# cunningham-lab/cyclic-gps

Measured on AMD Instinct MI355X. Metric: block-tridiag solve+log-det (mahal_and_det) algorithmic GB/s vs HBM roofline, N=2^20 d=4 on one GPU, N=2^24 d=4 time-axis sharded on several; solves/s alongside, higher is better.
Workload: dtype f64; 1 GPU; BASELINE config 2: mahal_and_det on ONE SPD block-tridiagonal system, N=1048576 block rows (1048576 per GPU), d=4, conditioned bidiagonal-factor generator seed 1234; rows_total=1048576, rows_per_gpu=1048576, d=4, algorithmic_bytes=301989776, parallelism=single GPU, algo=tile-fused

## Files before the change

### cyclic-gps_amd/csrc/cgps_tile.h

```cpp
#pragma once
#include <cstdlib>
#include <map>
#include <mutex>
#include <utility>
#include <type_traits>

#include "cgps_level.h"
#include "cgps_plan.h"
#include "cgps_leg.h"

namespace cgps {
#include "cgps_tile_leg.h"

template <typename T, int D>
struct LdsTile {
  static constexpr int DD = D * D;
  static constexpr int VN = Vec16<T>::N;
  static constexpr int G = (DD % VN == 0) ? DD / VN : 0;
  static constexpr bool SWZ = G >= 2 && (G & (G - 1)) == 0;
  T* R;
  T* Oc;
  T* y;
  static __device__ __forceinline__ int key(int row) { return (row ^ (row >> 3) ^ (row >> 6) ^ (row >> 9)) & (G - 1); }

// ... 280 lines not shown
          }
        }
      }
      CGPS_STAMP(1);
      __syncthreads();
      CGPS_STAMP(2);
      if (act) {
        if (role == 0) {
          LT::store_blk(t.R, e, W);
          store_vec<T, D>(t.y + e * D, wv);
        } else if (role == 1) {
          LT::store_blk(t.R, o, W);
          store_vec<T, D>(t.y + o * D, wv);
        } else if (role == 2) {
          LT::template store_rows<0, DH>(t.Oc, e - s + 1, W);
        } else {
          LT::template store_rows<DH, D>(t.Oc, e - s + 1, W);
        }
      }
      __syncthreads();
      CGPS_STAMP(3);
      ++stamp_pass;
    }
  }
  return levels;
}

template <typename T>
__device__ __forceinline__ void store_wt(T* p, T v) {
  __hip_atomic_store(p, v, __ATOMIC_RELAXED, __HIP_MEMORY_SCOPE_AGENT);
}
template <bool COH, typename T>
__device__ __forceinline__ T load_coh(const T* p) {
  if constexpr (COH) return __hip_atomic_load(const_cast<T*>(p), __ATOMIC_RELAXED, __HIP_MEMORY_SCOPE_AGENT);
  else return *p;
}
template <bool COH, typename T>
__device__ __forceinline__ typename Vec16<T>::type load16_coh(const T* p) {
  using V = typename Vec16<T>::type;
  if constexpr (COH) {
    unsigned long long* q = reinterpret_cast<unsigned long long*>(const_cast<T*>(p));
    unsigned long long w[2];
    w[0] = __hip_atomic_load(q, __ATOMIC_RELAXED, __HIP_MEMORY_SCOPE_AGENT);
    w[1] = __hip_atomic_load(q + 1, __ATOMIC_RELAXED, __HIP_MEMORY_SCOPE_AGENT);
    V v;
    __builtin_memcpy(&v, w, 16);
    return v;
  } else {
    return *reinterpret_cast<const V*>(p);
  }
}

constexpr int FOLD_SLOTS = 1024;
#ifndef CGPS_FOLD_GROUP
#define CGPS_FOLD_GROUP 16
#endif
constexpr int FOLD_GROUP = CGPS_FOLD_GROUP;
constexpr int FOLD_MAX_GROUPS = 64;
static __device__ unsigned int g_fold_counter[FOLD_SLOTS][1 + FOLD_MAX_GROUPS];

template <typename T, int D> constexpr int record_rcmax() { return (D == 8 || (sizeof(T) == 8 && D == 6)) ? 1 : 4; }

template <typename T, int D>
struct RecordLayout {
  static constexpr int DD = D * D;
  static constexpr int STRIDE = record_stride(D);
  static constexpr int RS = 0, CS = DD, DRA = 2 * DD, YS = 3 * DD, DYA = 3 * DD + D;
};


template <typename T, int D>
__device__ __forceinline__ void collect_left_updates(LdsTile<T, D>& t, int levels, T (&dRa)[D][D], T (&dya)[D]) {
  for (int l = 0; l < levels; ++l) {
    const int slot = (1 << l) - 1;
    T P[D][D], p[D];
    LdsTile<T, D>::load_blk(t.R, slot, P);
    load_vec<T, D>(t.y + slot * D, p);
#pragma unroll
    for (int i = 0; i < D; ++i) {
      dya[i] -= p[i];
#pragma unroll
      for (int j = 0; j <= i; ++j) dRa[i][j] -= P[i][j];
    }
  }
}

constexpr int FAIL_LATE = 0x40000000;
__device__ __forceinline__ int fail_code(bool early, bool any, int64_t row) {
  const int r = (int)(row < (int64_t)(FAIL_LATE - 2) ? row : (int64_t)(FAIL_LATE - 2)) + 1;
  return early ? r : (any ? (r | FAIL_LATE) : 0);
}
template <int NT>
__device__ __forceinline__ void write_partial(double mah, double logp, int failrow_plus1, double* __restrict__ partial,
                                              double* red, int* sfail) {
  if (failrow_plus1) atomicMin(sfail, failrow_plus1);
  block_sum2<NT>(mah, logp, red);
  if constexpr (NT <= 64) __syncthreads();
  if (threadIdx.x == 0) {
    double* p = partial;
    const int f = *sfail;
    store_wt(p + 0, mah);
    store_wt(p + 1, logp);
    store_wt(p + 2, (f == 0x7fffffff) ? 0.0 : (double)f);
    store_wt(p + 3, 0.0);
  }
}
// ... 105 lines not shown
    for (int l = 0; l < levels; ++l) {
      const int slot = (1 << l) - 1;
      dra -= elem(t.R, slot);
      dyv -= t.y[slot * D + i];
    }
    T* r = rec_out;
    store_wt(r + RL::RS + tid, elem(t.R, n_real - 1));
    store_wt(r + RL::CS + tid, elem(t.Oc, 0));
    store_wt(r + RL::DRA + tid, dra);
    if (j == 0) {
      store_wt(r + RL::YS + i, t.y[(n_real - 1) * D + i]);
      store_wt(r + RL::DYA + i, dyv);
    }
  }
}

template <typename T, int D, int NTILE, int NT>
struct StageSmem {
  static constexpr int DD = D * D;
  LdsTile<T, D> t;
  double* red;
  T* xch;
  int* sfail;
  __device__ __forceinline__ StageSmem(char* smem) {
    t.carve(smem, NTILE);
    char* tail = smem + ((((size_t)NTILE * (2 * DD + D) + DD) * sizeof(T) + 15) & ~(size_t)15);
    red = reinterpret_cast<double*>(tail);
    xch = reinterpret_cast<T*>(red + 2 * (NT / 64));
    sfail = reinterpret_cast<int*>(xch + (NT / 64) * (DD + D));
  }
};


template <typename T, int D> constexpr int stage1_row_group() {
  if (sizeof(T) == 8 && (D == 3 || D == 5)) return 2;
  return 1;
}
template <typename T, int D> constexpr int stage1_min_waves() {
  return ((sizeof(T) == 8 && D <= 4) || (sizeof(T) == 4 && D <= 5)) ? 2 : 1;
}
struct FoldArgs {
  int slot;
  void* group_records;
  double* out2;
  int* info;
  void* shard_record;
  double* shard_partial;
  int rows_per_lane;
  int pair_slot;
  size_t pair_ws_stride;
  const unsigned char* obs_pattern;
  int obs_entries;
};
template <typename T, int D, int NTILE, int NT, bool FINAL, bool INL = false>
__device__ __forceinline__ void record_reduce_body(char* smem, unsigned tile_index, const T* __restrict__ rin, int64_t n,
                                                   int rc, T* __restrict__ rout, double* __restrict__ partial_out,
                                                   const double* __restrict__ partial_in, int64_t n_partial,
                                                   double* __restrict__ out2, int* __restrict__ info,
                                                   int64_t rows_per_record, int64_t N, int64_t rstride, int64_t pstride);
template <typename T, int D, int NW, bool ONE_PER_CU>
__device__ __forceinline__ void fold_record_stages(char* smem, int* last_flag, T* __restrict__ rec, double* __restrict__ partial,
                                                   const FoldArgs& fold, int64_t rows_per_tile, int64_t N) {
  const int tid = threadIdx.x;
    constexpr bool COH = ONE_PER_CU && (D * D) % Vec16<T>::N == 0;
    using RL = RecordLayout<T, D>;
    const unsigned grp = blockIdx.x / FOLD_GROUP, ngrp = (gridDim.x + FOLD_GROUP - 1) / FOLD_GROUP;
    const unsigned gsize = (grp + 1 < ngrp) ? (unsigned)FOLD_GROUP : gridDim.x - grp * FOLD_GROUP;
    auto arrive = [&](unsigned int* ctr, unsigned expected) {
      if (tid < 64) {
        asm volatile("s_waitcnt vmcnt(0)" ::: "memory");
        if (tid == 0) {
          const bool last = atomicInc(ctr, expected - 1u) == expected - 1u;
          *last_flag = last ? 1 : 0;
          if (!COH && last) {
            __builtin_amdgcn_fence(__ATOMIC_ACQUIRE, "agent");
            asm volatile("s_waitcnt vmcnt(0)" ::: "memory");
          }
        }
      }
      __syncthreads();
      return *last_flag != 0;
    };
    T* grec = reinterpret_cast<T*>(fold.group_records);
    double* gpartial = partial + PARTIAL_STRIDE * (size_t)gridDim.x;
    const bool lead = arrive(&g_fold_counter[fold.slot][1 + grp], gsize);
    CGPS_KSTAMP(4);
    if (gridDim.x == 1) {
      record_reduce_body<T, D, FOLD_MAX_GROUPS, NW, true, COH>(smem, 0u, rec, (int64_t)1, 1, (T*)nullptr, (double*)nullptr,
                                                               partial, (int64_t)1, fold.out2, fold.info, rows_per_tile, N,
                                                               (int64_t)RL::STRIDE, (int64_t)PARTIAL_STRIDE);
      return;
    }
    if (lead) {
      record_reduce_body<T, D, FOLD_GROUP, NW, false, COH>(smem, grp, rec, (int64_t)gridDim.x, 1, grec, gpartial,
                                                           (const double*)nullptr, (int64_t)0, (double*)nullptr,
                                                           (int*)nullptr, rows_per_tile, N, (int64_t)RL::STRIDE,
                                                           (int64_t)PARTIAL_STRIDE);
      CGPS_KSTAMP(5);
      const bool fin = arrive(&g_fold_counter[fold.slot][0], ngrp);
      CGPS_KSTAMP(6);
      if (fin) {
        if (fold.shard_record != nullptr)
          record_reduce_body<T, D, FOLD_MAX_GROUPS, NW, false, COH>(smem, 0u, grec, (int64_t)ngrp, 1,
                                                                    reinterpret_cast<T*>(fold.shard_record), fold.shard_partial,
                                                                    partial, (int64_t)gridDim.x + ngrp, (double*)nullptr,
                                                                    (int*)nullptr, rows_per_tile * FOLD_GROUP, N,
                                                                    (int64_t)RL::STRIDE, (int64_t)PARTIAL_STRIDE);
        else
          record_reduce_body<T, D, FOLD_MAX_GROUPS, NW, true, COH>(smem, 0u, grec, (int64_t)ngrp, 1, (T*)nullptr,
                                                                   (double*)nullptr, partial, (int64_t)gridDim.x + ngrp,
                                                                   fold.out2, fold.info, rows_per_tile * FOLD_GROUP, N,
                                                                   (int64_t)RL::STRIDE, (int64_t)PARTIAL_STRIDE);
        CGPS_KSTAMP(7);
      }
    }
}

template <typename T, int D, int CT, int NT, int NW = NT, bool FOLD = false, int SRC = 0>
__global__ __launch_bounds__(NW, (NW > NT ? 1 : stage1_min_waves<T, D>())) void chunk_reduce_kernel(const T* __restrict__ Rg, const T* __restrict__ Og,
                                                          const T* __restrict__ yg, int64_t N,
                                                          const T* __restrict__ Oleft,
                                                          T* __restrict__ rec, double* __restrict__ partial,
                                                          FoldArgs fold) {
  constexpr int DD = D * D;
  extern __shared__ __attribute__((aligned(16))) char smem[];
  StageSmem<T, D, NT, NW> sm(smem);
  const int tid = threadIdx.x;
  CGPS_KSTAMP(0);
  if (tid == 0) *sm.sfail = 0x7fffffff;
  const int C = CT > 0 ? CT : fold.rows_per_lane;
  if constexpr (SRC >= 1) {
    if (blockIdx.y == 1) {
      Oleft = nullptr;
      yg = nullptr;
      rec = reinterpret_cast<T*>(reinterpret_cast<char*>(rec) + fold.pair_ws_stride);
      partial = reinterpret_cast<double*>(reinterpret_cast<char*>(partial) + fold.pair_ws_stride);
      fold.group_records = reinterpret_cast<char*>(fold.group_records) + fold.pair_ws_stride;
      fold.slot = fold.pair_slot;
      fold.out2 += 2;
      fold.info += 1;
    }
  }
  const int64_t lane0 = (int64_t)blockIdx.x * NT;
  const int64_t gl = lane0 + tid;
  int64_t r0 = gl * C, rE = gl * C + C;
  if (tid >= NT) r0 = N;
  const bool whole_chunk = rE <= N;
  const bool whole_chunk_and_next = rE <= N - 1;
  if (rE > N) rE = N;
  const int L = r0 < N ? (int)(rE - r0) : 0;
  PivotLog pl;
  double mah = 0.0;
// ... 403 lines not shown
    (void)hipFuncSetAttribute(reinterpret_cast<const void*>(&chunk_reduce_ml_kernel<T, D, Cfg::C, Cfg::NT1, Cfg::LPR, true>),
                              hipFuncAttributeMaxDynamicSharedMemorySize, lds1);
  }
  else if constexpr (Cfg::ALWAYS_WIDE) {
    const int ldsw = (int)stage_lds_bytes<T, D>(Cfg::NG1, 2 * Cfg::NT1);
    (void)hipFuncSetAttribute(reinterpret_cast<const void*>(&chunk_reduce_kernel<T, D, Cfg::C, Cfg::NT1, 2 * Cfg::NT1>),
                              hipFuncAttributeMaxDynamicSharedMemorySize, ldsw);
    (void)hipFuncSetAttribute(reinterpret_cast<const void*>(&chunk_reduce_kernel<T, D, Cfg::C, Cfg::NT1, 2 * Cfg::NT1, true>),
                              hipFuncAttributeMaxDynamicSharedMemorySize, ldsw);
    (void)hipFuncSetAttribute(reinterpret_cast<const void*>(&chunk_reduce_kernel<T, D, 0, Cfg::NT1, 2 * Cfg::NT1, true>),
                              hipFuncAttributeMaxDynamicSharedMemorySize, ldsw);
    (void)hipFuncSetAttribute(reinterpret_cast<const void*>(&chunk_reduce_kernel<T, D, 0, Cfg::NT1, 2 * Cfg::NT1, true, 1>),
                              hipFuncAttributeMaxDynamicSharedMemorySize, ldsw);
  } else {
    (void)hipFuncSetAttribute(reinterpret_cast<const void*>(&chunk_reduce_kernel<T, D, 0, Cfg::NT1, Cfg::NT1, true>),
                              hipFuncAttributeMaxDynamicSharedMemorySize, lds1);
    (void)hipFuncSetAttribute(reinterpret_cast<const void*>(&chunk_reduce_kernel<T, D, 0, Cfg::NT1, Cfg::NT1, true, 1>),
                              hipFuncAttributeMaxDynamicSharedMemorySize, lds1);
    (void)hipFuncSetAttribute(reinterpret_cast<const void*>(&chunk_reduce_kernel<T, D, Cfg::C, Cfg::NT1>),
                              hipFuncAttributeMaxDynamicSharedMemorySize, lds1);
    (void)hipFuncSetAttribute(reinterpret_cast<const void*>(&chunk_reduce_kernel<T, D, Cfg::C, Cfg::NT1, Cfg::NT1, true>),
                              hipFuncAttributeMaxDynamicSharedMemorySize, lds1);
    if constexpr (stage1_min_waves<T, D>() == 2) {
      (void)hipFuncSetAttribute(reinterpret_cast<const void*>(&chunk_reduce_kernel<T, D, Cfg::C, Cfg::NT1, 2 * Cfg::NT1>),
                                hipFuncAttributeMaxDynamicSharedMemorySize,
                                (int)stage_lds_bytes<T, D>(Cfg::NG1, 2 * Cfg::NT1));
      (void)hipFuncSetAttribute(reinterpret_cast<const void*>(&chunk_reduce_kernel<T, D, Cfg::C, Cfg::NT1, 2 * Cfg::NT1, true>),
                                hipFuncAttributeMaxDynamicSharedMemorySize,
                                (int)stage_lds_bytes<T, D>(Cfg::NG1, 2 * Cfg::NT1));
      (void)hipFuncSetAttribute(reinterpret_cast<const void*>(&chunk_reduce_kernel<T, D, 0, Cfg::NT1, 2 * Cfg::NT1, true>),
                                hipFuncAttributeMaxDynamicSharedMemorySize,
                                (int)stage_lds_bytes<T, D>(Cfg::NG1, 2 * Cfg::NT1));
    }
    (void)hipFuncSetAttribute(reinterpret_cast<const void*>(&chunk_reduce_kernel<T, D, 8, Cfg::NT1>),
                              hipFuncAttributeMaxDynamicSharedMemorySize, lds1);
    (void)hipFuncSetAttribute(reinterpret_cast<const void*>(&chunk_reduce_kernel<T, D, 8, Cfg::NT1, Cfg::NT1, true>),
                              hipFuncAttributeMaxDynamicSharedMemorySize, lds1);
    (void)hipFuncSetAttribute(reinterpret_cast<const void*>(&chunk_reduce_kernel<T, D, 4, Cfg::NT1>),
                              hipFuncAttributeMaxDynamicSharedMemorySize, lds1);
    (void)hipFuncSetAttribute(reinterpret_cast<const void*>(&chunk_reduce_kernel<T, D, 4, Cfg::NT1, Cfg::NT1, true>),
                              hipFuncAttributeMaxDynamicSharedMemorySize, lds1);
    (void)hipFuncSetAttribute(reinterpret_cast<const void*>(&chunk_reduce_kernel<T, D, 1, Cfg::NT1>),
                              hipFuncAttributeMaxDynamicSharedMemorySize, lds1);
    (void)hipFuncSetAttribute(reinterpret_cast<const void*>(&chunk_reduce_kernel<T, D, 1, Cfg::NT1, Cfg::NT1, true>),
                              hipFuncAttributeMaxDynamicSharedMemorySize, lds1);
  }
  (void)hipFuncSetAttribute(reinterpret_cast<const void*>(&record_reduce_kernel<T, D, Cfg::NTILE3, Cfg::NT3, false>),
                            hipFuncAttributeMaxDynamicSharedMemorySize, lds3);
  (void)hipFuncSetAttribute(reinterpret_cast<const void*>(&record_reduce_kernel<T, D, Cfg::NTILE3, Cfg::NT3, true>),
                            hipFuncAttributeMaxDynamicSharedMemorySize, lds3);
  });
}

static int fold_slot_for(const void* ws) {
  static std::mutex mu;
  static std::map<std::pair<int, const void*>, int> slots;
  static std::pair<int, const void*> owner[FOLD_SLOTS];
  static unsigned long long last_use[FOLD_SLOTS];
  static unsigned long long tick = 0;
  int dev = 0;
  (void)hipGetDevice(&dev);
  const std::pair<int, const void*> key{dev, ws};
  std::lock_guard<std::mutex> lock(mu);
  auto it = slots.find(key);
  int s;
  if (it != slots.end()) {
    s = it->second;
  } else if ((int)slots.size() < FOLD_SLOTS) {
    s = (int)slots.size();
    slots.emplace(key, s);
    owner[s] = key;
  } else {
    s = 0;
    for (int k = 1; k < FOLD_SLOTS; ++k)
      if (last_use[k] < last_use[s]) s = k;
    slots.erase(owner[s]);
    slots.emplace(key, s);
    owner[s] = key;
  }
  last_use[s] = ++tick;
  return s;
}
static hipError_t fold_reset_counters(hipStream_t st) {
  void* p = nullptr;
  hipError_t e = hipGetSymbolAddress(&p, HIP_SYMBOL(g_fold_counter));
  if (e != hipSuccess) return e;
  return hipMemsetAsync(p, 0, sizeof(unsigned int) * FOLD_SLOTS * (1 + FOLD_MAX_GROUPS), st);
}
inline bool fold_final_enabled() {
  static const bool on = [] { const char* e = getenv("CGPS_NO_FOLD"); return !(e && e[0] == '1'); }();
  return on;
}

inline int long_chunk_target_tiles() {
  static const int v = [] {
    const char* e = getenv("CGPS_S1_LONG");
    if (e && e[0] == '0') return 0;
    const char* t = getenv("CGPS_S1_TILES");
    const int n = t ? atoi(t) : 0;
    return n > 0 ? n : (int)STAGE1_SMALL_TILES;
  }();
  return v;
}
inline bool long_chunk_narrow() {
  static const bool on = [] { const char* e = getenv("CGPS_S1_NARROW"); return e && e[0] == '1'; }();
  return on;
}
inline int long_chunk_rows_per_lane(int64_t N, int lanes, int c_full, int block_bytes) {
  const int tiles = long_chunk_target_tiles();
  if (tiles <= 0) return 0;
  static const int forced = [] { const char* e = getenv("CGPS_S1_C"); return e ? atoi(e) : 0; }();
  if (forced > 0 && forced % 4 == 0 && (N + (int64_t)forced * lanes - 1) / ((int64_t)forced * lanes) <= 1024 &&
      N > (int64_t)forced * lanes)
    return forced;
  const int64_t per_round = (int64_t)tiles * lanes;
  int64_t c = (N + per_round - 1) / per_round;
  c = (c + 3) & ~(int64_t)3;
  if (c <= c_full || c > (1 << 20)) return 0;
  if (c * block_bytes > 2048 && c * block_bytes < 16384) return 0;
  return (int)c;
}

template <typename T, int D>
int run_tile_mahal_logdet(const T* Rs, const T* Os, const T* x, int64_t N, char* ws, size_t ws_bytes, double* out2,
                          int* info, hipStream_t st, hipEvent_t ev_start = nullptr, hipEvent_t ev_stop = nullptr,
                          const T* Oleft = nullptr, T* shard_record = nullptr, double* shard_partial = nullptr) {
  using Cfg = TileCfg<T, D>;
  using RL = RecordLayout<T, D>;
  static_assert(Cfg::ROWS1 == tile_rows1(D, sizeof(T)), "the workspace is sized for other stage-1 tiles than the kernels take");
  const cgps_host::TileWs w = cgps_host::tile_ws(N, D, sizeof(T));
  if (ws_bytes < w.total) return -1;
  const int clong = (Cfg::LPR > 1 || !fold_final_enabled()) ? 0 : long_chunk_rows_per_lane(N, Cfg::NG1, Cfg::C, (int)(D * D * sizeof(T)));
  const int csel = clong > 0 ? clong : ((Cfg::LPR > 1 || Cfg::ALWAYS_WIDE) ? Cfg::C : stage1_rows_per_lane(N, Cfg::C, Cfg::NT1));
  const int64_t rows_per_tile = (int64_t)csel * Cfg::NG1;
// ... 197 lines not shown
```

### cyclic-gps_amd/csrc/dev_bench.hip

```cpp
#include <hip/hip_runtime.h>

#include <cmath>
#include <cstdio>
#include <cstdlib>
#include <vector>

#define CGPS_FIN_STAMPS 1
#ifndef DEVB_D
#define DEVB_D 4
#endif
#ifndef DEVB_T
#define DEVB_T double
#endif
#include "cgps_tile.h"

using namespace cgps;

template <typename T, int D>
__device__ __forceinline__ void set_identity(T (&A)[D][D]) {
#pragma unroll
  for (int i = 0; i < D; ++i)
#pragma unroll
    for (int j = 0; j < D; ++j) A[i][j] = (i == j) ? T(1) : T(0);
}
// ... 145 lines not shown
        for (int b = 0; b <= a; ++b) { T v = (a == b) ? (T)2.5 + (T)0.2 * rnd() : (T)0.1 * rnd(); R[a][b] = v; R[b][a] = v; }
        for (int b = 0; b < D; ++b) O[a][b] = (T)0.3 * rnd();
        y[a] = rnd();
      }
      LdsTile<T, D>::store_blk(sm.t.R, tid, R);
      LdsTile<T, D>::store_blk(sm.t.Oc, tid, O);
      store_vec<T, D>(sm.t.y + tid * D, y);
    }
    __syncthreads();
    const long long t0 = wall_clock64();
    tile_cr<T, D, NTHR, MW>(sm.t, n_real, pl, mah, fail);
    const long long t1 = wall_clock64();
    __syncthreads();
    acc += t1 - t0;
  }
  double logp = pl.value();
  block_sum2<NTHR>(mah, logp, sm.red);
  if (tid == 0) {
    ticks[blockIdx.x] = acc;
    sums[2 * blockIdx.x] = mah;
    sums[2 * blockIdx.x + 1] = logp;
  }
}

template <int NTHR, int MW>
void run_tilecr(int grid, hipStream_t st) {
  const size_t lds = stage_lds_bytes<DEVB_T, DEVB_D>(256, NTHR);
  CK(hipFuncSetAttribute(reinterpret_cast<const void*>(&tilecr_bench_kernel<NTHR, MW>),
                         hipFuncAttributeMaxDynamicSharedMemorySize, (int)lds));
  long long* ticks;
  double* sums;
  CK(hipMalloc(&ticks, grid * sizeof(long long)));
  CK(hipMalloc(&sums, 2 * grid * sizeof(double)));
  const int reps = 50;
  printf("tile_cr NTHR=%d MW=%d grid=%d :", NTHR, MW, grid);
  double prev = 0;
  for (int n_real : {2, 4, 8, 16, 32, 64, 128, 256}) {
    hipLaunchKernelGGL((tilecr_bench_kernel<NTHR, MW>), dim3(grid), dim3(NTHR), lds, st, n_real, reps, ticks, sums);
    CK(hipStreamSynchronize(st));
    std::vector<long long> h(grid);
    std::vector<double> hs(2 * grid);
    CK(hipMemcpy(h.data(), ticks, grid * sizeof(long long), hipMemcpyDeviceToHost));
    CK(hipMemcpy(hs.data(), sums, 2 * grid * sizeof(double), hipMemcpyDeviceToHost));
    double avg = 0;
    for (auto v : h) avg += (double)v;
    avg = avg / grid / reps * 10.0;
    printf("  n=%d: %.0f ns (+%.0f)", n_real, avg, avg - prev);
    if (n_real == 256) printf("  [check %.10g %.10g]", hs[0], hs[1]);
    prev = avg;
  }
  printf("\n");
  CK(hipFree(ticks));
  CK(hipFree(sums));
}

template <typename F>
float time_ms(F&& launch, int reps, hipStream_t st) {
  hipEvent_t a, b;
  CK(hipEventCreate(&a));
  CK(hipEventCreate(&b));
  launch();
  CK(hipStreamSynchronize(st));
  CK(hipEventRecord(a, st));
  for (int i = 0; i < reps; ++i) launch();
  CK(hipEventRecord(b, st));
  CK(hipEventSynchronize(b));
  float ms = 0;
  CK(hipEventElapsedTime(&ms, a, b));
  CK(hipGetLastError());
  return ms / reps;
}

template <typename T, int D, int C, int NT>
void run_chunk_variants(const T* R, const T* O, const T* y, int64_t N, double* out, hipStream_t st, double bytes) {
  const int64_t tiles = (N + (int64_t)C * NT - 1) / ((int64_t)C * NT);
  float a = time_ms([&] { hipLaunchKernelGGL((loads_only_kernel<T, D, C, NT>), dim3((unsigned)tiles), dim3(NT), 0, st, R, O, y, N, out); }, 20, st);
  float b = time_ms([&] { hipLaunchKernelGGL((chunk_only_kernel<T, D, C, NT>), dim3((unsigned)tiles), dim3(NT), 0, st, R, O, y, N, out); }, 20, st);
  printf("C=%2d NT=%3d tiles=%6lld : loads-only %7.2f us (%5.2f TB/s)   chunk-only %7.2f us (%5.2f TB/s)\n", C, NT,
         (long long)tiles, a * 1e3, bytes / (a * 1e-3) / 1e12, b * 1e3, bytes / (b * 1e-3) / 1e12);
}

int main(int argc, char** argv) {
  using T = double;
  constexpr int D = DEVB_D;
  const int lg = argc > 1 ? atoi(argv[1]) : 20;
  const int64_t N = (int64_t)1 << lg;
  if (argc > 2 && atoi(argv[2]) == 2) {
    hipStream_t s2;
    CK(hipStreamCreate(&s2));
    T *R2, *O2, *y2;
    CK(hipMalloc(&R2, N * D * D * sizeof(T)));
    CK(hipMalloc(&O2, N * D * D * sizeof(T)));
    CK(hipMalloc(&y2, N * D * sizeof(T)));
    hipLaunchKernelGGL((gen_kernel<T, D>), dim3((unsigned)((N + 255) / 256)), dim3(256), 0, s2, R2, O2, y2, N);
    const size_t wsb = cgps_host::tile_ws(N, D, sizeof(T)).total;
    char* ws;
    double* out2;
    int* info;
    CK(hipMalloc(&ws, wsb));
    CK(hipMalloc(&out2, 16));
    CK(hipMalloc(&info, 4));
    for (int mode = (argc > 3 ? atoi(argv[3]) : 0); mode < 2; ++mode) {
      setenv("CGPS_NO_FOLD", mode == 0 ? "1" : "0", 1);
      for (int it = 0; it < 30; ++it) {
        hipEvent_t ea, eb;
        CK(hipEventCreate(&ea));
        CK(hipEventCreate(&eb));
        CK(hipEventRecord(ea, s2));
        int rc = run_tile_mahal_logdet<T, D>(R2, O2, y2, N, ws, wsb, out2, info, s2);
        CK(hipEventRecord(eb, s2));
        CK(hipStreamSynchronize(s2));
        float ms;
        CK(hipEventElapsedTime(&ms, ea, eb));
        long long st[16];
        CK(hipMemcpyFromSymbol(st, HIP_SYMBOL(g_fin_stamps), sizeof(st)));
        double o[2];
        CK(hipMemcpy(o, out2, 16, hipMemcpyDeviceToHost));
        if (it >= 28) {
          static long long ks[512][12];
          CK(hipMemcpyFromSymbol(ks, HIP_SYMBOL(g_k_stamps), sizeof(ks)));
          long long t0 = ks[0][0];
          for (int b = 0; b < 256; ++b) t0 = ks[b][0] < t0 ? ks[b][0] : t0;
          static int xcc[512];
          CK(hipMemcpyFromSymbol(xcc, HIP_SYMBOL(g_k_xcc), sizeof(xcc)));
          double sx[8] = {0}, mx[8] = {0};
          int cx[8] = {0};
          for (int b = 0; b < 256; ++b) {
            const int x = xcc[b] & 7;
            const double d = (ks[b][1] - t0) * 0.01;
            sx[x] += d; cx[x]++; mx[x] = d > mx[x] ? d : mx[x];
          }
          printf("   stream end per XCD (avg/max us):");
          for (int x = 0; x < 8; ++x) printf(" [%d: n=%d %.1f/%.1f]", x, cx[x], cx[x] ? sx[x] / cx[x] : 0.0, mx[x]);
          printf("\n   stream end by block index (us):");
          for (int b = 0; b < 256; b += 17) printf(" b%d:%.1f", b, (ks[b][1] - t0) * 0.01);
          printf("\n");
          const char* names[10] = {"start", "streamed", "tile reduced+emitted", "partial written", "arrived(group)",
                                   "group reduced", "arrived(top)", "final done", "rows staged in LDS", "tile_cr done"};
          for (int k = 0; k < 10; ++k) {
            long long lo = 1LL << 62, hi = 0;
            int cnt = 0;
            for (int b = 0; b < 256; ++b) {
              if (ks[b][k] < t0) continue;
              lo = ks[b][k] < lo ? ks[b][k] : lo;
              hi = ks[b][k] > hi ? ks[b][k] : hi;
              ++cnt;
            }
            if (cnt) printf("   %-22s first %.2f us  last %.2f us  (%d workgroups)\n", names[k], (lo - t0) * 0.01, (hi - t0) * 0.01, cnt);
          }
        }
        if (it >= 27)
          printf("mode %s rc %d: op %.1f us | final: loads %.2f  lds-stores %.2f  reduce %.2f  last-row %.2f  sums+write %.2f  total %.2f us  [%.10g %.10g]\n",
                 mode == 0 ? "two launches" : "folded", rc, ms * 1e3, (st[1] - st[0]) * 0.01, (st[2] - st[1]) * 0.01,
                 (st[3] - st[2]) * 0.01, (st[4] - st[3]) * 0.01, (st[5] - st[4]) * 0.01, (st[5] - st[0]) * 0.01, o[0], o[1]);
      }
      break;
    }
    return 0;
  }
  if (argc > 2 && atoi(argv[2]) == 1) {
    hipStream_t s2;
    CK(hipStreamCreate(&s2));
    for (int grid : {1, 256}) {
      run_tilecr<256, 1>(grid, s2);
      run_tilecr<256, 2>(grid, s2);
      run_tilecr<256, 4>(grid, s2);
      run_tilecr<512, 1>(grid, s2);
      run_tilecr<512, 2>(grid, s2);
      run_tilecr<512, 4>(grid, s2);
    }
    return 0;
  }
  hipStream_t st;
  CK(hipStreamCreate(&st));
  T *R, *O, *y;
  double* out;
  CK(hipMalloc(&R, N * D * D * sizeof(T)));
  CK(hipMalloc(&O, N * D * D * sizeof(T)));
  CK(hipMalloc(&y, N * D * sizeof(T)));
  CK(hipMalloc(&out, 4096));
  hipLaunchKernelGGL((gen_kernel<T, D>), dim3((unsigned)((N + 255) / 256)), dim3(256), 0, st, R, O, y, N);
  CK(hipStreamSynchronize(st));
  const double bytes = ((2.0 * N - 1) * D * D + N * D) * sizeof(T);
  printf("N=2^%d d=%d fp64  algorithmic bytes %.1f MB\n", lg, D, bytes / 1e6);
  run_mfma_probe();

  {
    const int64_t n16 = N * D * D * sizeof(T) / 16;
    float ms = time_ms([&] {
      hipLaunchKernelGGL(coalesced_read_kernel, dim3(2048), dim3(256), 0, st, (const double2*)R, n16, out);
      hipLaunchKernelGGL(coalesced_read_kernel, dim3(2048), dim3(256), 0, st, (const double2*)O, n16, out);
    }, 20, st);
    printf("coalesced read of R+O (2 launches): %7.2f us  (%5.2f TB/s)\n", ms * 1e3, 2.0 * n16 * 16 / (ms * 1e-3) / 1e12);
  }
  run_chunk_variants<T, D, 4, 256>(R, O, y, N, out, st, bytes);
  run_chunk_variants<T, D, 8, 256>(R, O, y, N, out, st, bytes);
  run_chunk_variants<T, D, 16, 256>(R, O, y, N, out, st, bytes);
  run_chunk_variants<T, D, 8, 128>(R, O, y, N, out, st, bytes);
  run_chunk_variants<T, D, 8, 64>(R, O, y, N, out, st, bytes);
  run_chunk_variants<T, D, 16, 64>(R, O, y, N, out, st, bytes);
  run_chunk_variants<T, D, 32, 64>(R, O, y, N, out, st, bytes);

  return 0;
}
```

Before: 4375 GB/s.

## Fold f64 d=4 record reduction stages in one wave using registers and DPP

For double precision with d=4 and at most 256 workgroups, the cross-workgroup fold of per-tile records now runs in a single 64-lane wave. The block-tridiagonal cyclic reduction over up to 16 records is done in registers with MFMA 4x4 ops and DPP row rotations, replacing the LDS-staged multi-wave reduction. The aim is to shorten the serial tail latency of the last-arriving workgroups, at the cost of considerable new index-mapping complexity. An environment variable falls back to the LDS path, and a microbenchmark mode is added.

```diff
diff --git a/cyclic-gps_amd/csrc/cgps_tile.h b/cyclic-gps_amd/csrc/cgps_tile.h
--- a/cyclic-gps_amd/csrc/cgps_tile.h
+++ b/cyclic-gps_amd/csrc/cgps_tile.h
@@ -356,6 +356,7 @@
 }
 
 constexpr int FOLD_SLOTS = 1024;
+constexpr int FOLD_SLOT_LDS_STAGES = 1 << 16;
 #ifndef CGPS_FOLD_GROUP
 #define CGPS_FOLD_GROUP 16
 #endif
@@ -567,6 +568,7 @@
   const unsigned char* obs_pattern;
   int obs_entries;
 };
+#include "cgps_tile_rec.h"
 template <typename T, int D, int NTILE, int NT, bool FINAL, bool INL = false>
 __device__ __forceinline__ void record_reduce_body(char* smem, unsigned tile_index, const T* __restrict__ rin, int64_t n,
                                                    int rc, T* __restrict__ rout, double* __restrict__ partial_out,
@@ -581,6 +583,51 @@
     using RL = RecordLayout<T, D>;
     const unsigned grp = blockIdx.x / FOLD_GROUP, ngrp = (gridDim.x + FOLD_GROUP - 1) / FOLD_GROUP;
     const unsigned gsize = (grp + 1 < ngrp) ? (unsigned)FOLD_GROUP : gridDim.x - grp * FOLD_GROUP;
+    const int slot = fold.slot & (FOLD_SLOT_LDS_STAGES - 1);
+    if constexpr (std::is_same<T, double>::value && D == 4 && FOLD_GROUP == fold_reg::MAX_RECORDS) {
+      if (gridDim.x <= FOLD_GROUP * fold_reg::MAX_RECORDS && !(fold.slot & FOLD_SLOT_LDS_STAGES)) {
+        if (tid >= 64) return;
+        int lane = tid;
+        asm volatile("" : "+v"(lane));
+        auto arrive1 = [&](unsigned int* ctr, unsigned expected) {
+          asm volatile("s_waitcnt vmcnt(0)" ::: "memory");
+          int last = 0;
+          if (lane == 0) last = atomicInc(ctr, expected - 1u) == expected - 1u;
+          last = __builtin_amdgcn_readfirstlane(last);
+          if (!COH && last) {
+            __builtin_amdgcn_fence(__ATOMIC_ACQUIRE, "agent");
+            asm volatile("s_waitcnt vmcnt(0)" ::: "memory");
+          }
+          return last != 0;
+        };
+        const double* recd = reinterpret_cast<const double*>(rec);
+        double* grecd = reinterpret_cast<double*>(fold.group_records);
+        double* gpart = partial + PARTIAL_STRIDE * (size_t)gridDim.x;
+        const bool lead1 = arrive1(&g_fold_counter[slot][1 + grp], gsize);
+        CGPS_KSTAMP(4);
+        if (!lead1) return;
+        const bool single = gridDim.x == 1;
+#pragma unroll 1
+        for (int top = single ? 1 : 0; top < 2; ++top) {
+          const bool t1 = top != 0;
+          const double* rin = t1 ? (single ? recd : grecd) : recd + (size_t)grp * FOLD_GROUP * RL::STRIDE;
+          double* rout = t1 ? reinterpret_cast<double*>(fold.shard_record) : grecd + (size_t)grp * RL::STRIDE;
+          double* pout = t1 ? fold.shard_partial : gpart + PARTIAL_STRIDE * (size_t)grp;
+          const int n = t1 ? (single ? 1 : (int)ngrp) : (int)gsize;
+          const int np = t1 ? (single ? 1 : (int)(gridDim.x + ngrp)) : 0;
+          record_stage_reg<COH>(lane, t1 && fold.shard_record == nullptr, rin, n, rout, pout, t1 ? partial : nullptr, np,
+                                fold.out2, fold.info, t1 ? (int64_t)0 : (int64_t)grp * FOLD_GROUP,
+                                (t1 && !single) ? rows_per_tile * FOLD_GROUP : rows_per_tile, N);
+          if (t1) break;
+          CGPS_KSTAMP(5);
+          const bool fin1 = arrive1(&g_fold_counter[slot][0], ngrp);
+          CGPS_KSTAMP(6);
+          if (!fin1) return;
+        }
+        CGPS_KSTAMP(7);
+        return;
+      }
+    }
     auto arrive = [&](unsigned int* ctr, unsigned expected) {
       if (tid < 64) {
         asm volatile("s_waitcnt vmcnt(0)" ::: "memory");
@@ -598,7 +645,7 @@
     };
     T* grec = reinterpret_cast<T*>(fold.group_records);
     double* gpartial = partial + PARTIAL_STRIDE * (size_t)gridDim.x;
-    const bool lead = arrive(&g_fold_counter[fold.slot][1 + grp], gsize);
+    const bool lead = arrive(&g_fold_counter[slot][1 + grp], gsize);
     CGPS_KSTAMP(4);
     if (gridDim.x == 1) {
       record_reduce_body<T, D, FOLD_MAX_GROUPS, NW, true, COH>(smem, 0u, rec, (int64_t)1, 1, (T*)nullptr, (double*)nullptr,
@@ -612,7 +659,7 @@
                                                            (int*)nullptr, rows_per_tile, N, (int64_t)RL::STRIDE,
                                                            (int64_t)PARTIAL_STRIDE);
       CGPS_KSTAMP(5);
-      const bool fin = arrive(&g_fold_counter[fold.slot][0], ngrp);
+      const bool fin = arrive(&g_fold_counter[slot][0], ngrp);
       CGPS_KSTAMP(6);
       if (fin) {
         if (fold.shard_record != nullptr)
@@ -1122,6 +1169,11 @@
   });
 }
 
+inline bool fold_reg_enabled() {
+  static const bool on = [] { const char* e = getenv("CGPS_FOLD_REG"); return !(e && e[0] == '0'); }();
+  return on;
+}
+
 static int fold_slot_for(const void* ws) {
   static std::mutex mu;
   static std::map<std::pair<int, const void*>, int> slots;
@@ -1149,7 +1201,7 @@
     owner[s] = key;
   }
   last_use[s] = ++tick;
-  return s;
+  return fold_reg_enabled() ? s : (s | FOLD_SLOT_LDS_STAGES);
 }
 static hipError_t fold_reset_counters(hipStream_t st) {
   void* p = nullptr;
diff --git a/cyclic-gps_amd/csrc/cgps_tile_rec.h b/cyclic-gps_amd/csrc/cgps_tile_rec.h
--- /dev/null
+++ b/cyclic-gps_amd/csrc/cgps_tile_rec.h
@@ -0,0 +1,332 @@
+#pragma once
+
+namespace fold_reg {
+constexpr int MAX_RECORDS = 16;
+constexpr int set_of_residue(int m) { return m == 1 ? 2 : (m == 2 ? 1 : m); }
+constexpr int reg_set(int p) { return set_of_residue(p & 3); }
+constexpr int reg_blk(int p) { return p >> 2; }
+constexpr int position(int u, int b) { return 4 * b + set_of_residue(u); }
+constexpr int owner_lane(int p, int r, int c) { return 16 * r + 4 * reg_blk(p) + c; }
+constexpr int levels(int n) { int l = 0; while ((1 << l) < n) ++l; return l; }
+constexpr bool eliminated(int p, int l, int n) { return p < n - 1 && ((p + 1) & ((2 << l) - 1)) == (1 << l); }
+constexpr bool survivor(int p, int l) { return ((p + 1) & ((2 << l) - 1)) == 0; }
+constexpr bool right_is_tail(int p, int l, int n) { return p + (1 << l) >= n - 1; }
+constexpr bool left_is_outside(int p, int l) { return p < (1 << l); }
+constexpr int left_source(int p, int l) { return p - (1 << l); }
+constexpr int right_source(int p, int l) { return p + (1 << l); }
+constexpr int chains(int l) { return l == 0 ? 2 : 1; }
+constexpr int chain_set(int l, int j) { return l == 0 ? j : (l == 1 ? 2 : 3); }
+constexpr int right_set(int l, int u) { return l == 0 ? u + 2 : 3; }
+constexpr int right_rot(int l, int u) { return l == 2 ? 4 : (l == 3 ? 8 : 0); }
+constexpr int left_set(int l, int u) { return l == 0 ? 3 - u : 3; }
+constexpr int left_rot(int l, int u) { return (l == 0 && u == 1) ? 0 : (l == 3 ? 8 : 12); }
+constexpr int last_eliminated(int l, int n) { return ((n - 1 - (1 << l)) / (2 << l)) * (2 << l) + (1 << l) - 1; }
+}
+
+#ifdef __HIPCC__
+template <int ROT>
+__device__ __forceinline__ double row_rot_f64(double v) {
+  static_assert(ROT >= 1 && ROT <= 15, "row_ror:1..15");
+  const int lo = __builtin_amdgcn_mov_dpp(__double2loint(v), 0x120 + ROT, 0xf, 0xf, false);
+  const int hi = __builtin_amdgcn_mov_dpp(__double2hiint(v), 0x120 + ROT, 0xf, 0xf, false);
+  return __hiloint2double(hi, lo);
+}
+__device__ __forceinline__ double sum_over_b(double v) {
+  v += row_rot_f64<4>(v);
+  return v + row_rot_f64<8>(v);
+}
+
+template <int U>
+struct RecElim {
+  double GGt[U], Gx[U], FFt[U], Fx[U], FGt[U], GFt[U], X[U], piv[U];
+  bool f[U];
+};
+template <int U, bool PRODUCTS = true>
+__device__ __forceinline__ void rec_eliminate(int r, double ident, double (&A)[U], const double (&Ol)[U],
+                                              const double (&OrT)[U], const double (&Y)[U], RecElim<U>& o) {
+  double B[U];
+#pragma unroll
+  for (int u = 0; u < U; ++u) { B[u] = ident; o.piv[u] = 1.0; o.f[u] = false; }
+#pragma unroll
+  for (int kk = 0; kk < 4; ++kk) {
+    const double sel = (r == kk) ? 1.0 : 0.0;
+    double rowA[U], rowB[U], p[U], col[U];
+#pragma unroll
+    for (int u = 0; u < U; ++u) {
+      rowA[u] = mfma444(sel, A[u], 0.0);
+      rowB[u] = mfma444(sel, B[u], 0.0);
+    }
+#pragma unroll
+    for (int u = 0; u < U; ++u) {
+      if (kk == 0) { p[u] = quad_bcast_f64<0>(rowA[u]); col[u] = quad_bcast_f64<0>(A[u]); }
+      else if (kk == 1) { p[u] = quad_bcast_f64<1>(rowA[u]); col[u] = quad_bcast_f64<1>(A[u]); }
+      else if (kk == 2) { p[u] = quad_bcast_f64<2>(rowA[u]); col[u] = quad_bcast_f64<2>(A[u]); }
+      else { p[u] = quad_bcast_f64<3>(rowA[u]); col[u] = quad_bcast_f64<3>(A[u]); }
+      o.f[u] = o.f[u] || !(p[u] > 0.0);
+      o.piv[u] *= p[u];
+    }
+    double rs[U];
+#pragma unroll
+    for (int u = 0; u < U; ++u) rs[u] = rsqrt_fast(p[u]);
+#pragma unroll
+    for (int u = 0; u < U; ++u) {
+      const double lik = col[u] * rs[u];
+      const double ra = rowA[u] * rs[u], rb = rowB[u] * rs[u];
+      if (r > kk) {
+        A[u] = __builtin_fma(-lik, ra, A[u]);
+        B[u] = __builtin_fma(-lik, rb, B[u]);
+      } else if (r == kk) {
+        B[u] = rb;
+      }
+    }
+  }
+  double Um[U], Gt[U], Ft[U];
+#pragma unroll
+  for (int u = 0; u < U; ++u) Um[u] = mfma444(B[u], ident, 0.0);
+#pragma unroll
+  for (int u = 0; u < U; ++u) {
+    o.X[u] = mfma444(Um[u], Y[u], 0.0);
+    if constexpr (PRODUCTS) {
+      Gt[u] = mfma444(Um[u], Ol[u], 0.0);
+      Ft[u] = mfma444(Um[u], OrT[u], 0.0);
+    }
+  }
+  if constexpr (PRODUCTS) {
+#pragma unroll
+    for (int u = 0; u < U; ++u) {
+      o.GGt[u] = mfma444(Gt[u], Gt[u], 0.0);
+      o.Gx[u] = mfma444(Gt[u], o.X[u], 0.0);
+      o.FFt[u] = mfma444(Ft[u], Ft[u], 0.0);
+      o.Fx[u] = mfma444(Ft[u], o.X[u], 0.0);
+      o.FGt[u] = mfma444(Ft[u], Gt[u], 0.0);
+      o.GFt[u] = mfma444(Gt[u], Ft[u], 0.0);
+    }
+  }
+}
+
+struct RecStage {
+  double R[4], Y[4], CL[4], CRt[4];
+  double RK, YK, CLK;
+  double dra, dya;
+  double mah;
+  PivotLog pl;
+  int fcode;
+};
+
+template <int L>
+__device__ __forceinline__ void rec_stage_level(RecStage& t, int K, int b, int r, int c, double ident, int64_t rec0,
+                                                int64_t rows_per_record, int64_t N) {
+  namespace fr = fold_reg;
+  constexpr int S = 1 << L, NU = fr::chains(L), MASK = 2 * S - 1;
+  double A[NU], Ol[NU], OrT[NU], Yv[NU];
+  bool act[NU], spec[NU];
+#pragma unroll
+  for (int j = 0; j < NU; ++j) {
+    const int u = fr::chain_set(L, j), p = fr::position(u, b);
+    act[j] = ((p + 1) & MASK) == S && p < K;
+    spec[j] = act[j] && p + S >= K;
+    A[j] = act[j] ? t.R[u] : ident;
+    Ol[j] = act[j] ? t.CL[u] : 0.0;
+    OrT[j] = act[j] ? t.CRt[u] : 0.0;
+    Yv[j] = act[j] ? t.Y[u] : 0.0;
+  }
+  RecElim<NU> e;
+  rec_eliminate<NU>(r, ident, A, Ol, OrT, Yv, e);
+#pragma unroll
+  for (int j = 0; j < NU; ++j) {
+    t.mah += e.X[j] * e.X[j];
+    if (act[j] && r == 0 && c == 0) t.pl.mul(e.piv[j]);
+    if (act[j] && e.f[j]) {
+      int64_t frow = (rec0 + fr::position(fr::chain_set(L, j), b) + 1) * rows_per_record;
+      frow = (frow < N ? frow : N) - 1;
+      const int code = fail_code(false, true, frow);
+      t.fcode = code < t.fcode ? code : t.fcode;
+    }
+  }
+  if (fr::last_eliminated(L, K + 1) + S >= K) {
+    double tR = 0.0, tY = 0.0, tC = 0.0;
+#pragma unroll
+    for (int j = 0; j < NU; ++j) {
+      tR += spec[j] ? e.FFt[j] : 0.0;
+      tY += spec[j] ? e.Fx[j] : 0.0;
+      tC += spec[j] ? e.FGt[j] : 0.0;
+    }
+    t.RK -= sum_over_b(tR);
+    t.YK -= sum_over_b(tY);
+    t.CLK = -sum_over_b(tC);
+  }
+  if (b == fr::reg_blk(S - 1)) {
+    t.dra += e.GGt[0];
+    t.dya += e.Gx[0];
+  }
+  if constexpr (L == 0) {
+    static_assert(fr::right_set(0, 0) == 2 && fr::right_set(0, 1) == 3 && fr::left_set(0, 1) == 2 && fr::left_set(0, 0) == 3, "");
+    static_assert(fr::right_rot(0, 0) == 0 && fr::right_rot(0, 1) == 0 && fr::left_rot(0, 1) == 0, "");
+    constexpr int ROT = fr::left_rot(0, 0);
+    const double gR = row_rot_f64<ROT>(e.GGt[0]), gY = row_rot_f64<ROT>(e.Gx[0]), gC = row_rot_f64<ROT>(e.GFt[0]);
+    t.R[2] -= e.FFt[0];
+    t.Y[2] -= e.Fx[0];
+    t.CL[2] = -e.FGt[0];
+    t.R[2] -= e.GGt[1];
+    t.Y[2] -= e.Gx[1];
+    if (fr::position(2, b) + S < K) t.CRt[2] = -e.GFt[1];
+    t.R[3] -= e.FFt[1];
+    t.Y[3] -= e.Fx[1];
+    t.CL[3] = -e.FGt[1];
+    if (b < 3) {
+      t.R[3] -= gR;
+      t.Y[3] -= gY;
+      if (fr::position(3, b) + S < K) t.CRt[3] = -gC;
+    }
+  } else if constexpr (L == 1) {
+    static_assert(fr::right_set(1, 2) == 3 && fr::left_set(1, 2) == 3 && fr::right_rot(1, 2) == 0, "");
+    constexpr int ROT = fr::left_rot(1, 2);
+    const double gR = row_rot_f64<ROT>(e.GGt[0]), gY = row_rot_f64<ROT>(e.Gx[0]), gC = row_rot_f64<ROT>(e.GFt[0]);
+    t.R[3] -= e.FFt[0];
+    t.Y[3] -= e.Fx[0];
+    t.CL[3] = -e.FGt[0];
+    if (b < 3) {
+      t.R[3] -= gR;
+      t.Y[3] -= gY;
+      if (fr::position(3, b) + S < K) t.CRt[3] = -gC;
+    }
+  } else if constexpr (L == 2) {
+    static_assert(fr::right_set(2, 3) == 3 && fr::left_set(2, 3) == 3, "");
+    constexpr int ROTL = fr::right_rot(2, 3), ROTR = fr::left_rot(2, 3);
+    const double fR = row_rot_f64<ROTL>(e.FFt[0]), fY = row_rot_f64<ROTL>(e.Fx[0]), fC = row_rot_f64<ROTL>(e.FGt[0]);
+    const double gR = row_rot_f64<ROTR>(e.GGt[0]), gY = row_rot_f64<ROTR>(e.Gx[0]), gC = row_rot_f64<ROTR>(e.GFt[0]);
+    if (b == 1) {
+      t.R[3] -= fR;
+      t.Y[3] -= fY;
+      t.CL[3] = -fC;
+      t.R[3] -= gR;
+      t.Y[3] -= gY;
+      if (fr::position(3, b) + S < K) t.CRt[3] = -gC;
+    }
+  }
+}
+
+__device__ __forceinline__ void rec_wave_reduce(double& a, double& b2, int& m) {
+#pragma unroll
+  for (int off = 32; off > 0; off >>= 1) {
+    a += __shfl_down(a, off, 64);
+    b2 += __shfl_down(b2, off, 64);
+    const int o = __shfl_down(m, off, 64);
+    m = o < m ? o : m;
+  }
+}
+
+constexpr int REC_STAGE_MAX_PARTIALS = 320;
+template <bool COH>
+__device__ __forceinline__ void record_stage_reg(int lane, bool FINAL, const double* rin, int n, double* rout,
+                                                 double* partial_out, const double* partial_in,
+                                                 int n_partial, double* out2, int* info,
+                                                 int64_t rec0, int64_t rows_per_record, int64_t N) {
+  using RL = RecordLayout<double, 4>;
+  namespace fr = fold_reg;
+  const int b = (lane >> 2) & 3, r = lane >> 4, c = lane & 3;
+  const int el = 4 * r + c, elT = 4 * c + r;
+  const double ident = (r == c) ? 1.0 : 0.0;
+  const bool c0 = (c == 0);
+  const int K = n - 1;
+  CGPS_FSTAMP(0);
+  double lR[4], lU[4], lC[4], lCr[4], lY[4], lYu[4];
+#pragma unroll
+  for (int u = 0; u < 4; ++u) {
+    const int p = fr::position(u, b);
+    const bool ok = p < K;
+    const double* q = rin + (size_t)(ok ? p : 0) * RL::STRIDE;
+    const double* q1 = rin + (size_t)(ok ? p + 1 : 0) * RL::STRIDE;
+    lR[u] = load_coh<COH>(q + RL::RS + el);
+    lU[u] = load_coh<COH>(q1 + RL::DRA + el);
+    lC[u] = load_coh<COH>(q + RL::CS + el);
+    lCr[u] = load_coh<COH>(q1 + RL::CS + elT);
+    lY[u] = load_coh<COH>(q + RL::YS + r);
+    lYu[u] = load_coh<COH>(q1 + RL::DYA + r);
+  }
+  const double* qk = rin + (size_t)K * RL::STRIDE;
+  const double kR = load_coh<COH>(qk + RL::RS + el), kC = load_coh<COH>(qk + RL::CS + el), kY = load_coh<COH>(qk + RL::YS + r);
+  const double oR = load_coh<COH>(rin + RL::DRA + el), oY = load_coh<COH>(rin + RL::DYA + r);
+  constexpr int PIT = REC_STAGE_MAX_PARTIALS / 64;
+  double pm[PIT], pg[PIT], pf[PIT];
+#pragma unroll
+  for (int it = 0; it < PIT; ++it) {
+    const int i = lane + 64 * it;
+    const bool ok = partial_in != nullptr && i < n_partial;
+    const double* p = (partial_in != nullptr ? partial_in : partial_out) + (size_t)PARTIAL_STRIDE * (ok ? i : 0);
+    pm[it] = ok ? load_coh<COH>(p) : 0.0;
+    pg[it] = ok ? load_coh<COH>(p + 1) : 0.0;
+    pf[it] = ok ? load_coh<COH>(p + 2) : 0.0;
+  }
+  CGPS_FSTAMP(1);
+  RecStage t;
+#pragma unroll
+  for (int u = 0; u < 4; ++u) {
+    const bool ok = fr::position(u, b) < K;
+    t.R[u] = ok ? lR[u] + lU[u] : ident;
+    t.Y[u] = (ok && c0) ? lY[u] + lYu[u] : 0.0;
+    t.CL[u] = ok ? lC[u] : 0.0;
+    t.CRt[u] = ok ? lCr[u] : 0.0;
+  }
+  t.RK = kR;
+  t.YK = c0 ? kY : 0.0;
+  t.CLK = kC;
+  t.dra = 0.0;
+  t.dya = 0.0;
+  t.mah = 0.0;
+  t.fcode = 0x7fffffff;
+  CGPS_FSTAMP(2);
+  if (K >= 1) rec_stage_level<0>(t, K, b, r, c, ident, rec0, rows_per_record, N);
+  if (K >= 2) rec_stage_level<1>(t, K, b, r, c, ident, rec0, rows_per_record, N);
+  if (K >= 4) rec_stage_level<2>(t, K, b, r, c, ident, rec0, rows_per_record, N);
+  if (K >= 8) rec_stage_level<3>(t, K, b, r, c, ident, rec0, rows_per_record, N);
+  CGPS_FSTAMP(3);
+  if (FINAL) {
+    double A[1] = {t.RK}, Z[1] = {0.0}, Yv[1] = {t.YK};
+    RecElim<1> e;
+    rec_eliminate<1, false>(r, ident, A, Z, Z, Yv, e);
+    if (b == 0) t.mah += e.X[0] * e.X[0];
+    if (lane == 0) t.pl.mul(e.piv[0]);
+    if (e.f[0]) {
+      const int code = fail_code(false, true, N - 1);
+      t.fcode = code < t.fcode ? code : t.fcode;
+    }
+    CGPS_FSTAMP(4);
+  } else {
+    const double dra = oR - sum_over_b(t.dra), dya = oY - sum_over_b(t.dya);
+    if (b == 0) {
+      store_wt(rout + RL::RS + el, t.RK);
+      store_wt(rout + RL::CS + el, t.CLK);
+      store_wt(rout + RL::DRA + el, dra);
+      if (c0) {
+        store_wt(rout + RL::YS + r, t.YK);
+        store_wt(rout + RL::DYA + r, dya);
+      }
+    }
+  }
+  double mah = t.mah, logp = t.pl.value();
+  int fcode = t.fcode;
+#pragma unroll
+  for (int it = 0; it < PIT; ++it) {
+    mah += pm[it];
+    logp += pg[it];
+    if (pf[it] != 0.0 && (int)pf[it] < fcode) fcode = (int)pf[it];
+  }
+  rec_wave_reduce(mah, logp, fcode);
+  if (lane == 0) {
+    const bool ok = (fcode == 0x7fffffff);
+    if (FINAL) {
+      const double poison = __builtin_nan("");
+      out2[0] = ok ? mah : poison;
+      out2[1] = ok ? logp : poison;
+      *info = ok ? 0 : (fcode & ~FAIL_LATE);
+    } else {
+      store_wt(partial_out + 0, mah);
+      store_wt(partial_out + 1, logp);
+      store_wt(partial_out + 2, ok ? 0.0 : (double)fcode);
+      store_wt(partial_out + 3, 0.0);
+    }
+  }
+  CGPS_FSTAMP(5);
+}
+#endif
diff --git a/cyclic-gps_amd/csrc/dev_bench.hip b/cyclic-gps_amd/csrc/dev_bench.hip
--- a/cyclic-gps_amd/csrc/dev_bench.hip
+++ b/cyclic-gps_amd/csrc/dev_bench.hip
@@ -221,6 +221,107 @@
   printf("\n");
   CK(hipFree(ticks));
   CK(hipFree(sums));
+}
+
+template <bool REG, bool FINAL>
+__global__ __launch_bounds__(512) void record_stage_bench_kernel(const double* rec, int n, int reps, double* rout, double* pout,
+                                                                 const double* pin, int n_partial, double* out2, int* info,
+                                                                 long long* ticks) {
+  extern __shared__ __attribute__((aligned(16))) char smem[];
+  using RL = RecordLayout<double, 4>;
+  long long acc = 0;
+  for (int rep = 0; rep < reps; ++rep) {
+    __syncthreads();
+    const long long t0 = wall_clock64();
+    if constexpr (REG) {
+      if (threadIdx.x < 64)
+        record_stage_reg<true>((int)threadIdx.x, FINAL, rec, n, rout, pout, FINAL ? pin : nullptr, FINAL ? n_partial : 0, out2, info,
+                                      0, 4096, (int64_t)n * 4096);
+    } else {
+      record_reduce_body<double, 4, (FINAL ? FOLD_MAX_GROUPS : FOLD_GROUP), 512, FINAL, true>(smem, 0u, rec, (int64_t)n, 1, rout, pout, FINAL ? pin : nullptr,
+                                                                  FINAL ? (int64_t)n_partial : 0, out2, info, 4096,
+                                                                  (int64_t)n * 4096, (int64_t)RL::STRIDE, (int64_t)PARTIAL_STRIDE);
+    }
+    asm volatile("s_waitcnt vmcnt(0)" ::: "memory");
+    const long long t1 = wall_clock64();
+    acc += t1 - t0;
+  }
+  if (threadIdx.x == 0) ticks[0] = acc;
+}
+
+template <bool REG, bool FINAL>
+static void run_record_stage(const double* rec, int n, double* rout, double* pout, const double* pin, int n_partial, double* out2,
+                             int* info, long long* ticks, hipStream_t st) {
+  using RL = RecordLayout<double, 4>;
+  const size_t lds = stage_lds_bytes<double, 4>(FOLD_MAX_GROUPS, 512);
+  const int reps = 200;
+  for (int pass = 0; pass < 2; ++pass)
+    hipLaunchKernelGGL((record_stage_bench_kernel<REG, FINAL>), dim3(1), dim3(512), lds, st, rec, n, reps, rout, pout, pin, n_partial,
+                       out2, info, ticks);
+  CK(hipStreamSynchronize(st));
+  long long t;
+  CK(hipMemcpy(&t, ticks, sizeof(t), hipMemcpyDeviceToHost));
+  double r[RL::STRIDE], p[4], o[2];
+  int inf;
+  CK(hipMemcpy(r, rout, sizeof(r), hipMemcpyDeviceToHost));
+  CK(hipMemcpy(p, pout, sizeof(p), hipMemcpyDeviceToHost));
+  CK(hipMemcpy(o, out2, sizeof(o), hipMemcpyDeviceToHost));
+  CK(hipMemcpy(&inf, info, sizeof(inf), hipMemcpyDeviceToHost));
+  double cs = 0;
+  for (int i = 0; i < RL::STRIDE; ++i) cs += r[i] * (1 + i);
+  if (FINAL)
+    printf("  %-9s top stage   n=%2d (+%3d partial results): %6.0f ns   [out2 %.15g %.15g info %d]\n", REG ? "registers" : "LDS", n,
+           n_partial, (double)t / reps * 10.0, o[0], o[1], inf);
+  else
+    printf("  %-9s group stage n=%2d: %6.0f ns   [record checksum %.15g partial %.15g %.15g %g]\n", REG ? "registers" : "LDS", n,
+           (double)t / reps * 10.0, cs, p[0], p[1], p[2]);
+}
+
+static void run_record_stages(hipStream_t st) {
+  using RL = RecordLayout<double, 4>;
+  constexpr int NREC = 16, NPART = 272;
+  std::vector<double> h((size_t)NREC * RL::STRIDE), hp((size_t)NPART * PARTIAL_STRIDE, 0.0);
+  unsigned s = 12345u;
+  auto rnd = [&]() { s = s * 1664525u + 1013904223u; return (double)((s >> 8) & 0xffff) / 65536.0 - 0.5; };
+  for (int w = 0; w < NREC; ++w) {
+    double* r = h.data() + (size_t)w * RL::STRIDE;
+    for (int a = 0; a < 4; ++a)
+      for (int b = 0; b <= a; ++b) {
+        const double v = (a == b) ? 2.5 + 0.2 * rnd() : 0.1 * rnd(), u = (a == b) ? -0.2 - 0.1 * rnd() : 0.02 * rnd();
+        r[RL::RS + 4 * a + b] = r[RL::RS + 4 * b + a] = v;
+        r[RL::DRA + 4 * a + b] = r[RL::DRA + 4 * b + a] = u;
+      }
+    for (int a = 0; a < 16; ++a) r[RL::CS + a] = 0.3 * rnd();
+    for (int a = 0; a < 4; ++a) { r[RL::YS + a] = rnd(); r[RL::DYA + a] = 0.1 * rnd(); }
+  }
+  for (int i = 0; i < NPART; ++i) { hp[(size_t)i * PARTIAL_STRIDE] = 1.0 + rnd(); hp[(size_t)i * PARTIAL_STRIDE + 1] = 3.0 + rnd(); }
+  double *rec, *rout, *pout, *pin, *out2;
+  int* info;
+  long long* ticks;
+  CK(hipMalloc(&rec, h.size() * sizeof(double)));
+  CK(hipMalloc(&rout, RL::STRIDE * sizeof(double)));
+  CK(hipMalloc(&pout, 4 * sizeof(double)));
+  CK(hipMalloc(&pin, hp.size() * sizeof(double)));
+  CK(hipMalloc(&out2, 2 * sizeof(double)));
+  CK(hipMalloc(&info, sizeof(int)));
+  CK(hipMalloc(&ticks, sizeof(long long)));
+  CK(hipMemcpy(rec, h.data(), h.size() * sizeof(double), hipMemcpyHostToDevice));
+  CK(hipMemcpy(pin, hp.data(), hp.size() * sizeof(double), hipMemcpyHostToDevice));
+  CK(hipMemset(rout, 0, RL::STRIDE * sizeof(double)));
+  CK(hipMemset(pout, 0, 4 * sizeof(double)));
+  CK(hipMemset(out2, 0, 2 * sizeof(double)));
+  CK(hipMemset(info, 0, sizeof(int)));
+  CK(hipFuncSetAttribute(reinterpret_cast<const void*>(&record_stage_bench_kernel<false, false>),
+                         hipFuncAttributeMaxDynamicSharedMemorySize, (int)stage_lds_bytes<double, 4>(FOLD_MAX_GROUPS, 512)));
+  CK(hipFuncSetAttribute(reinterpret_cast<const void*>(&record_stage_bench_kernel<false, true>),
+                         hipFuncAttributeMaxDynamicSharedMemorySize, (int)stage_lds_bytes<double, 4>(FOLD_MAX_GROUPS, 512)));
+  printf("one record stage, one workgroup of 512 threads, mean of 200 repetitions inside one launch\n");
+  for (int n : {16, 9, 2}) {
+    run_record_stage<false, false>(rec, n, rout, pout, pin, NPART, out2, info, ticks, st);
+    run_record_stage<true, false>(rec, n, rout, pout, pin, NPART, out2, info, ticks, st);
+    run_record_stage<false, true>(rec, n, rout, pout, pin, NPART, out2, info, ticks, st);
+    run_record_stage<true, true>(rec, n, rout, pout, pin, NPART, out2, info, ticks, st);
+  }
 }
 
 template <typename F>
@@ -327,6 +428,12 @@
     }
     return 0;
   }
+  if (argc > 2 && atoi(argv[2]) == 3) {
+    hipStream_t s3;
+    CK(hipStreamCreate(&s3));
+    run_record_stages(s3);
+    return 0;
+  }
   if (argc > 2 && atoi(argv[2]) == 1) {
     hipStream_t s2;
     CK(hipStreamCreate(&s2));
```

After: 4519 GB/s (median of 6 runs). 1.03x the previous value.
